# yanyan-li/PlanarSLAM

Hardware: AMD Instinct MI355X
Metric: RGB-D frames/sec (extract+match+pose-opt) @640x480; 1->8-GPU batch scaling (higher is better)
Workload: dtype u8/f64

## Files before the change

planarslam_amd/csrc/planepost.hip:

```cpp
#include "common.h"
#include "isort.h"

#include <algorithm>
#include <cmath>
#include <cstdlib>

namespace planar {
namespace planepost {

#ifndef PLANAR_PP_NT
#define PLANAR_PP_NT 512
#endif
constexpr int NT = PLANAR_PP_NT;
constexpr int MAXP = 128;
constexpr int NRNG = 32768;
constexpr int VOX_BIAS = 8192;
constexpr unsigned long long EMPTY = ~0ull;

struct Geo {
    int dev_skip_heap = 0;
    int pl_first = 0, pl_count = 1 << 20;
    int W, H, max_points, pl_stride, tcap, mini;
    float fx, fy, cx, cy, factor, leaf;
    double dist_th, log_probability, rfx, rfy;
    size_t ws_stride, off_cnt, off_cent, off_key, off_rank, off_vstart, off_pl, off_init, off_meta, off_ranges, off_blocks, off_heapj, off_items, off_dsort, off_gpos;
    int rows_long = 0, gpos_half = 0;
};

struct Pt { float x, y, z; };
__device__ __forceinline__ double mul_rcp(double n, double rd, bool& near) {
    const double t = n * rd;
    const int low = (int)((unsigned)__double_as_longlong(t) & 0x1fffffffu) - 0x10000000;
    near = low >= -8 && low <= 8;
    return t;
}
__device__ __forceinline__ Pt cam_point(const Geo& G, unsigned short d, int px, int py) {
    const double z = (double)d * (double)G.factor;
    const double nx = ((double)px - (double)G.cx) * z, ny = ((double)py - (double)G.cy) * z;
    bool near_x, near_y;
    double tx = mul_rcp(nx, G.rfx, near_x), ty = mul_rcp(ny, G.rfy, near_y);
    if (__ballot(near_x || near_y) != 0ull) {
        if (near_x) tx = nx / (double)G.fx;
        if (near_y) ty = ny / (double)G.fy;
    }
    return {(float)tx, (float)ty, (float)z};
}

__device__ __forceinline__ bool voxel_key(float x, float y, float z, float inv, unsigned plane, unsigned long long& key) {
    const int i0 = (int)floorf(x * inv) + VOX_BIAS, i1 = (int)floorf(y * inv) + VOX_BIAS, i2 = (int)floorf(z * inv) + VOX_BIAS;
    key = ((unsigned long long)plane << 42) | ((unsigned long long)(unsigned)i2 << 28) | ((unsigned long long)(unsigned)i1 << 14) | (unsigned long long)(unsigned)i0;
    return ((unsigned)i0 | (unsigned)i1 | (unsigned)i2) < 2u * VOX_BIAS;
}

__device__ __forceinline__ float red4(float a0, float a1, float a2, float a3) { return (a0 + a2) + (a1 + a3); }
__device__ __forceinline__ float plane_dot(const float m[4], float x, float y, float z) { return red4(m[0] * x, m[1] * y, m[2] * z, m[3] * 1.0f); }

__device__ __forceinline__ void roots2(float b, float c, float roots[3]) {
    roots[0] = 0.f;
    float d = (float)((double)(b * b) - 4.0 * (double)c);
    if (d < 0.0f) d = 0.0f;
    const float sd = sqrtf(d);
    roots[2] = 0.5f * (b + sd);
    roots[1] = 0.5f * (b - sd);
}
__device__ __forceinline__ void roots3(const float m[9], float roots[3]) {
    const float c0 = m[0] * m[4] * m[8] + 2.f * m[1] * m[2] * m[5] - m[0] * m[5] * m[5] - m[4] * m[2] * m[2] - m[8] * m[1] * m[1];
    const float c1 = m[0] * m[4] - m[1] * m[1] + m[0] * m[8] - m[2] * m[2] + m[4] * m[8] - m[5] * m[5];
    const float c2 = m[0] + m[4] + m[8];
    if (fabsf(c0) < 1.1920929e-07f) { roots2(c2, c1, roots); return; }
    const float s_inv3 = (float)(1.0 / 3.0), s_sqrt3 = sqrtf(3.0f);
    const float c2_over_3 = c2 * s_inv3;
    float a_over_3 = (c1 - c2 * c2_over_3) * s_inv3;
    if (a_over_3 > 0.f) a_over_3 = 0.f;
    const float half_b = 0.5f * (c0 + c2_over_3 * (2.f * c2_over_3 * c2_over_3 - c1));
    float q = half_b * half_b + a_over_3 * a_over_3 * a_over_3;
    if (q > 0.f) q = 0.f;
    const float rho = sqrtf(-a_over_3);
    const float theta = atan2f(sqrtf(-q), half_b) * s_inv3;
    const float cos_theta = cosf(theta), sin_theta = sinf(theta);
    roots[0] = c2_over_3 + 2.f * rho * cos_theta;
    roots[1] = c2_over_3 - rho * (cos_theta + s_sqrt3 * sin_theta);
    roots[2] = c2_over_3 - rho * (cos_theta - s_sqrt3 * sin_theta);
    float t;
    if (roots[0] >= roots[1]) { t = roots[0]; roots[0] = roots[1]; roots[1] = t; }
    if (roots[1] >= roots[2]) {
        t = roots[1]; roots[1] = roots[2]; roots[2] = t;
        if (roots[0] >= roots[1]) { t = roots[0]; roots[0] = roots[1]; roots[1] = t; }
    }
    if (roots[0] <= 0) roots2(c2, c1, roots);
}
__device__ __forceinline__ void eigen33_smallest(const float cov[9], float vec[3]) {
    float scale = 0.f;
#pragma unroll
    for (int k = 0; k < 9; k++) scale = fmaxf(scale, fabsf(cov[k]));
    if (scale <= 1.17549435e-38f) scale = 1.0f;
    float m[9];
#pragma unroll
    for (int k = 0; k < 9; k++) m[k] = cov[k] / scale;
    float roots[3];
    roots3(m, roots);
    m[0] -= roots[0]; m[4] -= roots[0]; m[8] -= roots[0];
    float v1[3], v2[3], v3[3];
    v1[0] = m[1] * m[5] - m[2] * m[4]; v1[1] = m[2] * m[3] - m[0] * m[5]; v1[2] = m[0] * m[4] - m[1] * m[3];
    v2[0] = m[1] * m[8] - m[2] * m[7]; v2[1] = m[2] * m[6] - m[0] * m[8]; v2[2] = m[0] * m[7] - m[1] * m[6];
    v3[0] = m[4] * m[8] - m[5] * m[7]; v3[1] = m[5] * m[6] - m[3] * m[8]; v3[2] = m[3] * m[7] - m[4] * m[6];
    const float l1 = v1[0] * v1[0] + (v1[1] * v1[1] + v1[2] * v1[2]), l2 = v2[0] * v2[0] + (v2[1] * v2[1] + v2[2] * v2[2]),
                l3 = v3[0] * v3[0] + (v3[1] * v3[1] + v3[2] * v3[2]);
    if (l1 >= l2 && l1 >= l3) { const float s = sqrtf(l1); vec[0] = v1[0] / s; vec[1] = v1[1] / s; vec[2] = v1[2] / s; }
    else if (l2 >= l1 && l2 >= l3) { const float s = sqrtf(l2); vec[0] = v2[0] / s; vec[1] = v2[1] / s; vec[2] = v2[2] / s; }
    else { const float s = sqrtf(l3); vec[0] = v3[0] / s; vec[1] = v3[1] / s; vec[2] = v3[2] / s; }
}

__device__ __forceinline__ int sac_plane(const Geo& G, const float* __restrict__ pts, int n, unsigned short* shuf, const int* __restrict__ rng, float coef[4], int* info) {
    const int lane = threadIdx.x & 63;
    auto wfence = [&]() { __builtin_amdgcn_fence(__ATOMIC_SEQ_CST, "wavefront"); __builtin_amdgcn_wave_barrier(); };
    for (int i = lane; i < n; i += 64) shuf[i] = (unsigned short)i;
    wfence();
    const double threshold = G.dist_th, one_over_indices = 1.0 / (double)n;
    int iterations = 0, best = -2147483647, draws = 0, bs0 = -1, bs1 = -1, bs2 = -1;
    double k = 1.0;
    unsigned skipped = 0;
    float bm[4] = {0.f, 0.f, 0.f, 0.f};
    bool have = false, exhausted = false;
    auto count_within = [&](const float m[4]) {
        int c = 0;
        for (int i0 = 0; i0 < n; i0 += 64) {
// ... 91 lines not shown
        cov[0] = a[0] - a[6] * a[6]; cov[1] = a[1] - a[6] * a[7]; cov[2] = a[2] - a[6] * a[8];
        cov[4] = a[3] - a[7] * a[7]; cov[5] = a[4] - a[7] * a[8]; cov[8] = a[5] - a[8] * a[8];
        cov[3] = cov[1]; cov[6] = cov[2]; cov[7] = cov[5];
        float v[3];
        eigen33_smallest(cov, v);
        refined[0] = v[0]; refined[1] = v[1]; refined[2] = v[2]; refined[3] = 0.f;
        refined[3] = -1 * red4(refined[0] * a[6], refined[1] * a[7], refined[2] * a[8], refined[3] * 1.0f);
    }
    const int nref = count_within(refined);
    if (info && lane == 0) { info[5] = n_inl; info[6] = nref; }
#pragma unroll
    for (int c = 0; c < 4; c++) coef[c] = refined[c];
    return nref != 0 ? 0 : 2;
}

__device__ __forceinline__ int max_point_distance(const Geo& G, float plane[4], const float* __restrict__ pts, int n, unsigned short* shuf, const int* __restrict__ rng, int* info) {
    const int lane = threadIdx.x & 63;
    bool far = false;
    for (int i0 = 0; i0 < n; i0 += 64) {
        const int i = i0 + lane;
        bool f = false;
        if (i < n) f = (double)fabsf(plane[0] * pts[i * 3] + plane[1] * pts[i * 3 + 1] + plane[2] * pts[i * 3 + 2] + plane[3]) > G.dist_th;
        far = far || (__ballot(f) != 0ull);
    }
    if (info && lane == 0) for (int c = 0; c < 12; c++) info[c] = c >= 2 && c <= 4 ? -1 : 0;
    if (far) return 1;
    float c[4];
    const int st = sac_plane(G, pts, n, shuf, rng, c, info);
    if (st) return st;
    const float oldVal = plane[3], newVal = c[3];
    const bool flip = (newVal < 0 && oldVal > 0) || (newVal > 0 && oldVal < 0);
#pragma unroll
    for (int t = 0; t < 4; t++) plane[t] = flip ? -c[t] : c[t];
    return 0;
}

__device__ __forceinline__ unsigned hash64(unsigned long long k) {
    k ^= k >> 33; k *= 0xff51afd7ed558ccdull; k ^= k >> 33;
    return (unsigned)k;
}

__device__ __forceinline__ void bitonic(unsigned long long* a, int n2) {
    for (int k = 2; k <= n2; k <<= 1)
        for (int j = k >> 1; j > 0; j >>= 1) {
            for (int t = threadIdx.x; t < n2 / 2; t += NT) {
                const int lo = ((t / j) * 2 * j) + (t % j), hi = lo + j;
                const bool up = (lo & k) == 0;
                const unsigned long long x = a[lo], y = a[hi];
                if ((x > y) == up) { a[lo] = y; a[hi] = x; }
            }
            __syncthreads();
        }
}

#ifndef PLANAR_WIDE_T
#define PLANAR_WIDE_T 1024
#endif
constexpr int PS_T = PLANAR_WIDE_T, PS_LT = 256, PS_E = 23, PS_SHIFT = 19, PS_R = 96;
constexpr int PS_HJOBS = 1024;
struct HeapClass { int max_len, cap, waves, wgs; };
constexpr HeapClass PS_HC[3] = {{2048, 2048, 4, 1}, {8192, 8192, 1, 2}, {1 << 30, 8192, 1, 4}};
using PsLds = isort::LdsLayout<PS_LT, PS_E>;
using PsGl = isort::GlobalLayout<PS_T>;
constexpr int PS_IT_SMALL = 256, PS_IT_BATCH = 256;
constexpr int ERR_SORT = 5;

struct Meta { int n_init, counts[2], err, M, npl, sort_status, heap_n, heap_n_global; };

__global__ __launch_bounds__(NT) void plane_voxels_kernel(Geo G, const unsigned short* __restrict__ depth_all, int pitch_px, long frame_stride_px,
                                                          const int* __restrict__ labels_all, const int* __restrict__ n_planes, unsigned char* ws_all, long long* timing) {
    extern __shared__ unsigned long long s_list[];
    __shared__ int s_first[MAXP], s_last[MAXP];
    __shared__ int s_n, s_err, s_kept, s_scan[NT / 64];
    const int b = blockIdx.x, tid = threadIdx.x, lane = tid & 63, wave = tid >> 6;
    const int HW = G.W * G.H;
    const unsigned short* D = depth_all + (size_t)b * frame_stride_px;
    const int* lab = labels_all + (size_t)b * HW;
    unsigned char* ws = ws_all + (size_t)b * G.ws_stride;
    unsigned* tcnt = (unsigned*)(ws + G.off_cnt);
    unsigned long long* gkey = (unsigned long long*)(ws + G.off_key);
    unsigned short* srank = (unsigned short*)(ws + G.off_rank);
    int* vstart = (int*)(ws + G.off_vstart);
    int* pfl = (int*)(ws + G.off_pl);
    isort::Range* init = (isort::Range*)(ws + G.off_init);
    Meta* meta = (Meta*)(ws + G.off_meta);
    int npl = n_planes[b];
    if (npl > MAXP) npl = MAXP;
    if (npl > G.pl_stride) npl = G.pl_stride;
    const float inv = 1.0f / G.leaf;
    const int TC = G.tcap;
    long long* tmark = timing ? timing + (size_t)b * 16 : nullptr;
    auto mark = [&](int q) { if (tmark && tid == 0) tmark[q] = wall_clock64(); };
    mark(0);

    for (int i = tid; i < TC; i += NT) { gkey[i] = EMPTY; tcnt[i] = 0u; }
    for (int i = tid; i < MAXP; i += NT) { s_first[i] = 0; s_last[i] = 0; }
    if (tid == 0) { s_n = 0; s_err = 0; s_kept = 0; }
    __threadfence();
    __syncthreads();

    mark(1);
    {
        constexpr int ROWS = 60, UNR = 4;
        const int MINI = G.mini;
        unsigned long long* mk = s_list + (size_t)wave * MINI;
        unsigned* mc = (unsigned*)(s_list + (size_t)(NT / 64) * MINI) + (size_t)wave * MINI;
        auto wfence = [&]() { __builtin_amdgcn_fence(__ATOMIC_SEQ_CST, "wavefront"); __builtin_amdgcn_wave_barrier(); };
        auto to_frame = [&](unsigned long long key, unsigned cnt) {
            unsigned h = hash64(key) & (unsigned)(TC - 1);
            for (int probe = 0; probe < TC; probe++) {
                const unsigned long long k = atomicCAS(&gkey[h], EMPTY, key);
                if (k == EMPTY) { if (atomicAdd(&s_n, 1) >= G.max_points) s_err = 3; }
                if (k == EMPTY || k == key) { atomicAdd(&tcnt[h], cnt); return; }
                h = (h + 1) & (unsigned)(TC - 1);
            }
            s_err = 3;
        };
        const int strips = (G.W + 63) / 64, tiles = strips * ((G.H + ROWS - 1) / ROWS);
        for (int tile = wave; tile < tiles; tile += NT / 64) {
            const int px = (tile % strips) * 64 + lane, y0 = (tile / strips) * ROWS, y1 = min(y0 + ROWS, G.H);
            const bool col = px < G.W;
            for (int e = lane; e < MINI; e += 64) { mk[e] = EMPTY; mc[e] = 0u; }
            wfence();
            unsigned long long cur = EMPTY, pend = EMPTY;
            unsigned cnt = 0, pcnt = 0;
            auto flush_parked = [&]() {
                if (pend != EMPTY) {
                    unsigned h = (hash64(pend) >> 7) & (unsigned)(MINI - 1);
                    bool done = false;
                    for (int probe = 0; probe < 8 && !done; probe++) {
                        const unsigned long long k = atomicCAS(&mk[h], EMPTY, pend);
                        if (k == EMPTY || k == pend) { atomicAdd(&mc[h], pcnt); done = true; }
                        h = (h + 1) & (unsigned)(MINI - 1);
                    }
                    if (!done) to_frame(pend, pcnt);
                    pend = EMPTY;
                }
            };
            int l4[UNR], ln[UNR];
            unsigned short d4[UNR], dn[UNR];
            const int pxc = min(px, G.W - 1);
            auto load = [&](int yb, int* l, unsigned short* d) {
#pragma unroll
                for (int q = 0; q < UNR; q++) {
                    const int yy = min(yb + q, G.H - 1);
                    const int lv = lab[(size_t)yy * G.W + pxc];
                    d[q] = D[(size_t)yy * pitch_px + pxc];
                    l[q] = (col && yb + q < y1) ? lv : -1;
                }
            };
            load(y0, l4, d4);
            for (int yb = y0; yb < y1; yb += UNR) {
                load(yb + UNR, ln, dn);
#pragma unroll
                for (int q = 0; q < UNR; q++) {
                    const int l = l4[q];
                    const bool on = l >= G.pl_first && l < npl && l - G.pl_first < G.pl_count;
                    unsigned long long key = cur;
                    bool fin = false;
                    const Pt p = cam_point(G, d4[q], px, yb + q);
                    if (on) {
                        if (!voxel_key(p.x, p.y, p.z, inv, (unsigned)l, key)) { s_err = 3; key = cur; }
                        fin = key != cur;
                    }
                    if (__ballot(fin && cur != EMPTY && pend != EMPTY) != 0ull) flush_parked();
                    if (fin) {
                        if (cur != EMPTY) { pend = cur; pcnt = cnt; }
                        cur = key; cnt = 0;
                    }
                    if (on && key == cur && cur != EMPTY) cnt++;
                }
#pragma unroll
                for (int q = 0; q < UNR; q++) { l4[q] = ln[q]; d4[q] = dn[q]; }
            }
            flush_parked();
            pend = cur; pcnt = cnt;
            flush_parked();
            wfence();
            for (int e = lane; e < MINI; e += 64)
                if (mk[e] != EMPTY) to_frame(mk[e], mc[e]);
            wfence();
        }
    }
    __threadfence();
    __syncthreads();
    const int err = s_err;
    const int M = err ? 0 : s_n;
    mark(2);

    if (!err) {
        int n2 = 64;
        while (n2 < M) n2 <<= 1;
        if (tid == 0) s_kept = 0;
        for (int i = M + tid; i < n2; i += NT) s_list[i] = EMPTY;
        __syncthreads();
        for (int i = tid; i < TC; i += NT) {
            const unsigned long long k = __hip_atomic_load(&gkey[i], __ATOMIC_RELAXED, __HIP_MEMORY_SCOPE_AGENT);
            if (k != EMPTY) s_list[atomicAdd(&s_kept, 1)] = (k << 14) | (unsigned long long)i;
        }
        __syncthreads();
        bitonic(s_list, n2);
        const int per = (M + NT - 1) / NT, r0 = min(M, tid * per), r1 = min(M, r0 + per);
        int mine = 0;
        for (int r = r0; r < r1; r++) {
            const unsigned long long e = s_list[r];
            const int s = (int)(e & 0x3fffull), p = (int)(e >> 56);
            srank[s] = (unsigned short)r;
            mine += (int)__hip_atomic_load(&tcnt[s], __ATOMIC_RELAXED, __HIP_MEMORY_SCOPE_AGENT);
            if (r == 0 || (int)(s_list[r - 1] >> 56) != p) s_first[p] = r;
            if (r == M - 1 || (int)(s_list[r + 1] >> 56) != p) s_last[p] = r + 1;
        }
        int total;
        int run = isort::block_exscan<NT, int>(mine, s_scan, &total);
        for (int r = r0; r < r1; r++) {
            vstart[r] = run;
            run += (int)__hip_atomic_load(&tcnt[(int)(s_list[r] & 0x3fffull)], __ATOMIC_RELAXED, __HIP_MEMORY_SCOPE_AGENT);
        }
        if (tid == 0) vstart[M] = total;
    }
    __threadfence();
    __syncthreads();
    for (int p = tid; p < MAXP; p += NT) { pfl[p] = s_first[p]; pfl[MAXP + p] = s_last[p]; }
    if (tid == 0) {
        int k = 0;
        for (int p = 0; p < npl && !err; p++) {
            if (s_last[p] <= s_first[p]) continue;
            const int f = vstart[s_first[p]], l = vstart[s_last[p]];
            init[k++] = isort::Range{f, l, isort::depth_limit(l - f)};
        }
        meta->n_init = k; meta->counts[0] = 0; meta->counts[1] = 0; meta->err = err; meta->M = M; meta->npl = npl; meta->sort_status = 0; meta->heap_n = 0; meta->heap_n_global = 0;
    }
    mark(3);
}

template <int SH, int IT>
__global__ __launch_bounds__(IT) void plane_items_kernel(Geo G, const unsigned short* __restrict__ depth_all, int pitch_px, long frame_stride_px,
                                                           const int* __restrict__ labels_all, unsigned char* ws_all) {
    constexpr int NW = IT / 64;
    __shared__ unsigned s_cnt[NW][MAXP];
    const int b = blockIdx.x, tid = threadIdx.x, lane = tid & 63, wave = tid >> 6;
    const int HW = G.W * G.H;
    unsigned char* ws = ws_all + (size_t)b * G.ws_stride;
    const Meta* meta = (const Meta*)(ws + G.off_meta);
    if (meta->err || meta->n_init == 0) return;
    const unsigned short* D = depth_all + (size_t)b * frame_stride_px;
    const int* lab = labels_all + (size_t)b * HW;
    const unsigned long long* gkey = (const unsigned long long*)(ws + G.off_key);
    const unsigned short* srank = (const unsigned short*)(ws + G.off_rank);
    const int* vstart = (const int*)(ws + G.off_vstart);
    const int* pfl = (const int*)(ws + G.off_pl);
    uint32_t* items = (uint32_t*)(ws + G.off_items);
    const int npl = meta->npl, TC = G.tcap;
    const float inv = 1.0f / G.leaf;
    for (int i = tid; i < NW * MAXP; i += IT) (&s_cnt[0][0])[i] = 0u;
    __syncthreads();
    const int S = ((HW + NW - 1) / NW + 63) & ~63, w0 = min(HW, wave * S), w1 = min(HW, w0 + S);
    auto wfence = [&]() { __builtin_amdgcn_fence(__ATOMIC_SEQ_CST, "wavefront"); __builtin_amdgcn_wave_barrier(); };
    constexpr int U = 4;
    for (int i0 = w0; i0 < w1; i0 += 64 * U) {
        int l[U];
#pragma unroll
        for (int u = 0; u < U; u++) l[u] = lab[min(i0 + 64 * u + lane, w1 - 1)];
#pragma unroll
        for (int u = 0; u < U; u++) {
            const bool on = i0 + 64 * u + lane < w1 && l[u] >= G.pl_first && l[u] < npl && l[u] - G.pl_first < G.pl_count;
            unsigned long long rem = __ballot(on);
            while (rem) {
                const int L = __builtin_amdgcn_readlane(l[u], __builtin_ctzll(rem));
                const unsigned long long m = __ballot(on && l[u] == L);
                if (lane == 0) s_cnt[wave][L] += (unsigned)__popcll(m);
                rem &= ~m;
            }
        }
    }
    __syncthreads();
    if (tid < npl) {
        const int first = pfl[tid], last = pfl[MAXP + tid];
        unsigned run = last > first ? (unsigned)vstart[first] : 0u;
        for (int w = 0; w < NW; w++) { const unsigned t = s_cnt[w][tid]; s_cnt[w][tid] = run; run += t; }
    }
    __syncthreads();
    for (int i0 = w0; i0 < w1; i0 += 64 * U) {
        int l[U];
        unsigned short d[U];
#pragma unroll
        for (int u = 0; u < U; u++) {
            const int pix = min(i0 + 64 * u + lane, w1 - 1), py = pix / G.W, px = pix - py * G.W;
            l[u] = lab[pix];
            d[u] = D[(size_t)py * pitch_px + px];
        }
#pragma unroll
        for (int u = 0; u < U; u++) {
            const int pix = i0 + 64 * u + lane, pc = min(pix, w1 - 1), py = pc / G.W, px = pc - py * G.W;
            const bool on = pix < w1 && l[u] >= G.pl_first && l[u] < npl && l[u] - G.pl_first < G.pl_count;
            const Pt p = cam_point(G, d[u], px, py);
            uint32_t item = 0;
            if (on) {
                unsigned long long key;
                voxel_key(p.x, p.y, p.z, inv, (unsigned)l[u], key);
                unsigned h = hash64(key) & (unsigned)(TC - 1);
                for (int probe = 0; probe < TC && gkey[h] != key; probe++) h = (h + 1) & (unsigned)(TC - 1);
                item = ((uint32_t)srank[h] << SH) | (uint32_t)pix;
            }
            unsigned long long rem = __ballot(on);
            while (rem) {
                const int L = __builtin_amdgcn_readlane(l[u], __builtin_ctzll(rem));
                const bool mine = on && l[u] == L;
                const unsigned long long m = __ballot(mine);
                const unsigned base = s_cnt[wave][L];
                wfence();
                if (mine) items[base + (unsigned)__popcll(m & ((1ull << lane) - 1ull))] = item;
                if (lane == 0) s_cnt[wave][L] = base + (unsigned)__popcll(m);
                wfence();
                rem &= ~m;
            }
        }
    }
}

template <int SH>
__global__ __launch_bounds__(PS_T) void plane_sort_global(Geo G, unsigned char* ws_all, int rows_cap) {
    extern __shared__ __align__(16) uint8_t sort_lds[];
    unsigned char* ws = ws_all + (size_t)blockIdx.x * G.ws_stride;
    Meta* meta = (Meta*)(ws + G.off_meta);
    if (meta->err || meta->n_init == 0) return;
    const isort::HeapSink HS{(isort::HeapJob*)(ws + G.off_heapj), &meta->heap_n, PS_HJOBS};
    isort::global_tier<SH, PS_T>((uint32_t*)(ws + G.off_items), (const isort::Range*)(ws + G.off_init), meta->n_init, PsLds::N, 64, (isort::Range*)(ws + G.off_ranges),
                                 (isort::Block*)(ws + G.off_blocks), isort::G_FMAX, meta->counts, sort_lds, rows_cap, HS, &meta->sort_status, 0xffffffffu,
                                 G.rows_long, G.rows_long ? (uint32_t*)(ws + G.off_gpos) : nullptr, G.gpos_half);
    __syncthreads();
    if (threadIdx.x == 0) meta->heap_n_global = min(meta->heap_n, PS_HJOBS);
}

constexpr int PS_EARLY = 4;
template <int SH>
__global__ __launch_bounds__(PS_LT, 4) void plane_sort_lds(Geo G, unsigned char* ws_all) {
    extern __shared__ __align__(16) uint8_t sort_lds[];
    unsigned char* ws = ws_all + (size_t)blockIdx.x * G.ws_stride;
    Meta* meta = (Meta*)(ws + G.off_meta);
    if (meta->err) return;
    if (blockIdx.y < PS_EARLY) {
        static_assert(PsLds::bytes >= PS_HC[2].cap * 4, "the early heap jobs keep the top PS_HC[2].cap words of a range in this workgroup's LDS");
        const int ng = meta->heap_n_global;
        if (threadIdx.x < 64 && ng > 0 && !G.dev_skip_heap)
            isort::heap_jobs<SH>((uint32_t*)(ws + G.off_items), (const isort::HeapJob*)(ws + G.off_heapj), ng, blockIdx.y, PS_EARLY, (uint32_t*)sort_lds, PS_HC[2].cap, 0, 1 << 30);
        return;
    }
    const isort::Range* ranges = (const isort::Range*)(ws + G.off_ranges);
    const isort::Block* blocks = (const isort::Block*)(ws + G.off_blocks);
    const int nb = meta->counts[1];
    const isort::HeapSink HS{(isort::HeapJob*)(ws + G.off_heapj), &meta->heap_n, PS_HJOBS};
    for (int k = blockIdx.y - PS_EARLY; k < nb; k += gridDim.y - PS_EARLY) {
        const isort::Block K = blocks[k];
        isort::lds_tier<SH, PS_LT, PS_E>((uint32_t*)(ws + G.off_items), ranges + K.r0, K.nr, K.f, K.l, sort_lds, HS, &meta->sort_status);
    }
}

template <int SH>
__global__ __launch_bounds__(256) void plane_sort_heap(Geo G, unsigned char* ws_all, int part, int min_len, int max_len, int cap) {
    extern __shared__ __align__(16) uint8_t sort_lds[];
    unsigned char* ws = ws_all + (size_t)blockIdx.x * G.ws_stride;
    const Meta* meta = (const Meta*)(ws + G.off_meta);
    const int ng = meta->heap_n_global, lo = part ? ng : 0, hi = meta->err ? 0 : (part ? min(meta->heap_n, PS_HJOBS) : ng), wave = threadIdx.x >> 6, nw = blockDim.x >> 6;
    if (hi > lo) isort::heap_jobs<SH>((uint32_t*)(ws + G.off_items), (const isort::HeapJob*)(ws + G.off_heapj) + lo, hi - lo, blockIdx.y * nw + wave, gridDim.y * nw,
                                           (uint32_t*)sort_lds + (size_t)wave * cap, cap, min_len, max_len);
}

__device__ __forceinline__ Pt cam_point_thread(const Geo& G, unsigned short d, int px, int py) {
    const double z = (double)d * (double)G.factor;
    const double nx = ((double)px - (double)G.cx) * z, ny = ((double)py - (double)G.cy) * z;
    bool near_x, near_y;
    double tx = mul_rcp(nx, G.rfx, near_x), ty = mul_rcp(ny, G.rfy, near_y);
    if (near_x) tx = nx / (double)G.fx;
    if (near_y) ty = ny / (double)G.fy;
    return {(float)tx, (float)ty, (float)z};
}

template <int SH>
__global__ __launch_bounds__(NT, 4) void plane_tail_kernel(Geo G, const unsigned short* __restrict__ depth_all, int pitch_px, long frame_stride_px,
                                                        const double* __restrict__ planes_all, int planes_stride, const int* __restrict__ rng, unsigned char* ws_all,
                                                        int* n_out, float* coef_out, int* src_out, int* off_out, float* pts_out, int* status, int* state_out,
                                                        int* nvox_out, int* info_out, long long* timing) {
    extern __shared__ unsigned long long s_list[];
    __shared__ int s_first[MAXP], s_last[MAXP], s_state[MAXP], s_k[MAXP], s_o[MAXP + 1];
    __shared__ float s_coef[MAXP][4];
    __shared__ int s_err, s_kept;
    const int b = blockIdx.x, tid = threadIdx.x, lane = tid & 63, wave = tid >> 6;
    const unsigned short* D = depth_all + (size_t)b * frame_stride_px;
    const double* planes = planes_all + (size_t)b * planes_stride * 8;
    unsigned char* ws = ws_all + (size_t)b * G.ws_stride;
    float* cent = (float*)(ws + G.off_cent);
    const int* vstart = (const int*)(ws + G.off_vstart);
    const int* pfl = (const int*)(ws + G.off_pl);
    const uint32_t* items = (const uint32_t*)(ws + G.off_items);
    const Meta* meta = (const Meta*)(ws + G.off_meta);
    const int npl = meta->npl;
    int err = meta->err ? meta->err : (meta->sort_status ? ERR_SORT : 0);
    const int M = err ? 0 : meta->M;
    long long* tmark = timing ? timing + (size_t)b * 16 : nullptr;
    auto mark = [&](int q) { if (tmark && tid == 0) tmark[q] = wall_clock64(); };
    for (int i = tid; i < MAXP; i += NT) { s_first[i] = pfl[i]; s_last[i] = pfl[MAXP + i]; s_state[i] = (i >= G.pl_first && i - G.pl_first < G.pl_count) ? 0 : 3; }
    if (tid == 0) { s_err = 0; s_kept = 0; }
    {
        unsigned short* dsort = (unsigned short*)(ws + G.off_dsort);
        const int total = M > 0 ? vstart[M] : 0;
        for (int i = tid; i < total; i += NT) {
            const int pix = (int)(items[i] & ((1u << SH) - 1u)), yy = pix / G.W;
            dsort[i] = D[(size_t)yy * pitch_px + (pix - yy * G.W)];
        }
        __threadfence_block();
        __syncthreads();
        for (int r = tid; r < M; r += NT) {
            const int i0 = vstart[r], i1 = vstart[r + 1];
            float cx = 0.f, cy = 0.f, cz = 0.f;
            constexpr int U = 16;
            for (int i = i0; i < i1; i += U) {
                uint32_t it[U];
                unsigned short d[U];
#pragma unroll
                for (int u = 0; u < U; u++) { it[u] = items[min(i + u, i1 - 1)]; d[u] = dsort[min(i + u, i1 - 1)]; }
#pragma unroll
                for (int u = 0; u < U; u++)
                    if (i + u < i1) {
                        const int pix = (int)(it[u] & ((1u << SH) - 1u)), yy = pix / G.W;
                        const Pt p = cam_point_thread(G, d[u], pix - yy * G.W, yy);
                        cx += p.x; cy += p.y; cz += p.z;
                    }
            }
            const float cnt = (float)(i1 - i0);
            cent[(size_t)r * 3] = cx / cnt; cent[(size_t)r * 3 + 1] = cy / cnt; cent[(size_t)r * 3 + 2] = cz / cnt;
        }
    }
    __threadfence();
    __syncthreads();

    mark(3);
    unsigned short* shuf = (unsigned short*)s_list;
    if (!err)
    for (int p = wave; p < npl; p += NT / 64) {
        if (s_state[p] != 0) continue;
        const double* P = planes + (size_t)p * 8;
        const double nx = P[1], ny = P[2], nz = P[3];
        float c[4] = {(float)nx, (float)ny, (float)nz, (float)-(nx * P[4] + ny * P[5] + nz * P[6])};
        const int first = s_first[p], n = s_last[p] - first;
        int* info = info_out ? info_out + ((size_t)b * G.pl_stride + p) * 12 : nullptr;
        const int st = max_point_distance(G, c, cent + (size_t)first * 3, n, shuf + first, rng, info);
        if (lane == 0) {
            s_state[p] = st;
#pragma unroll
            for (int t = 0; t < 4; t++) s_coef[p][t] = c[t];
            if (st == 4) s_err = 4;
        }
    }
    __syncthreads();
    if (!err) err = s_err;
    mark(4);

// ... 150 lines not shown
    const int* vstart = (const int*)(ws + G.off_vstart);
    const uint32_t* items = (const uint32_t*)(ws + G.off_items);
    const Meta* meta = (const Meta*)(ws + G.off_meta);
    const int err = meta->err ? meta->err : (meta->sort_status ? ERR_SORT : 0), M = err ? 0 : meta->M;
    for (int r = tid; r < M; r += NT) {
        const int i0 = vstart[r], i1 = vstart[r + 1];
        float cx = 0.f, cy = 0.f, cz = 0.f;
        for (int i = i0; i < i1; i++) { const int j = (int)(items[i] & ((1u << PS_SHIFT) - 1u)); cx += pts[j * 3]; cy += pts[j * 3 + 1]; cz += pts[j * 3 + 2]; }
        const float cnt = (float)(i1 - i0);
        out[(size_t)r * 3] = cx / cnt; out[(size_t)r * 3 + 1] = cy / cnt; out[(size_t)r * 3 + 2] = cz / cnt;
    }
    if (tid == 0) { *n_out = M; *status = err; }
}

static void sampler_table(std::vector<int>& tab) {
    std::vector<uint32_t> s(624);
    s[0] = 12345u;
    for (int i = 1; i < 624; i++) s[i] = 1812433253u * (s[i - 1] ^ (s[i - 1] >> 30)) + (uint32_t)i;
    int at = 624;
    tab.resize(NRNG);
    for (int q = 0; q < NRNG; q++) {
        if (at >= 624) {
            for (int i = 0; i < 624; i++) {
                const uint32_t y = (s[i] & 0x80000000u) | (s[(i + 1) % 624] & 0x7fffffffu);
                s[i] = s[(i + 397) % 624] ^ (y >> 1) ^ ((y & 1u) ? 0x9908b0dfu : 0u);
            }
            at = 0;
        }
        uint32_t y = s[at++];
        y ^= y >> 11; y ^= (y << 7) & 0x9d2c5680u; y ^= (y << 15) & 0xefc60000u; y ^= y >> 18;
        tab[q] = (int)(y >> 1);
    }
}

}
}

struct planar_plane_clouds {
    planar_ctx* ctx = nullptr;
    int max_batch = 0;
    planar::planepost::Geo G{};
    size_t smem = 0, smem_tail = 0, smem_cloud = 0, smem_sort_g = 0, smem_sort_l = 0;
    int sort_rows = 0, shift = 19;
    planar::DevBuf ws, rng, dbg;
    bool timing = false;
    std::vector<int32_t> last_status;
    planar::LaunchProfile prof{6};
};

using namespace planar;

extern "C" {

int planar_plane_clouds_create(planar_ctx* ctx, int width, int height, int max_batch, int max_points, planar_plane_clouds** out) {
    PLANAR_REQUIRE(ctx && out, PLANAR_EINVAL, "null argument");
    PLANAR_REQUIRE(width >= 16 && height >= 16 && width <= 4096 && height <= 4096 && max_batch >= 1, PLANAR_EINVAL, "bad size");
    PLANAR_REQUIRE(max_points >= 64 && max_points <= 8192 && (max_points & (max_points - 1)) == 0, PLANAR_EINVAL, "max_points must be a power of two in [64, 8192]");
    PLANAR_REQUIRE((long long)width * height <= (1ll << 20), PLANAR_EINVAL, "at most 2^20 pixels per frame (a sort word is voxel << 20 | pixel)");
    PLANAR_REQUIRE((long long)width * height <= (1ll << planepost::PS_SHIFT) || max_points <= 4096, PLANAR_EINVAL, "frames of more than 2^19 pixels take max_points <= 4096 (12 bits of voxel beside 20 bits of pixel)");
    PLANAR_HIP_CHECK(hipSetDevice(ctx->device));
    planar_plane_clouds* p = new planar_plane_clouds;
    p->ctx = ctx; p->max_batch = max_batch;
    planepost::Geo& G = p->G;
    G.W = width; G.H = height; G.max_points = max_points; G.pl_stride = planepost::MAXP;
    G.leaf = 0.1f; G.dist_th = 0.05;
    G.log_probability = std::log(1.0 - 0.99);
    G.tcap = 2 * max_points;
    {
        size_t off = 0;
        auto carve = [&](size_t bytes) { const size_t o = off; off = align_up(off + bytes, (size_t)256); return o; };
        G.off_cnt = carve((size_t)G.tcap * 4);
        G.off_key = carve((size_t)G.tcap * 8);
        G.off_rank = carve((size_t)G.tcap * 2);
        G.off_cent = carve((size_t)max_points * 12);
        G.off_vstart = carve((size_t)(max_points + 1) * 4);
        G.off_pl = carve((size_t)2 * planepost::MAXP * 4);
        G.off_init = carve((size_t)planepost::MAXP * sizeof(isort::Range));
        G.off_meta = carve(sizeof(planepost::Meta));
        G.off_ranges = carve((size_t)isort::G_FMAX * sizeof(isort::Range));
        G.off_blocks = carve((size_t)isort::G_FMAX * sizeof(isort::Block));
        G.off_heapj = carve((size_t)planepost::PS_HJOBS * sizeof(isort::HeapJob));
        G.off_items = carve(std::max((size_t)width * height, (size_t)65536) * 4);
        G.off_dsort = carve((size_t)width * height * 2);
        if (!planepost::PsGl::plan(std::max(width * height, 65536), p->sort_rows, G.rows_long)) { delete p; set_error("plane_clouds: frame too large for the sort's LDS-resident rank prefixes"); return PLANAR_EINVAL; }
        G.gpos_half = G.rows_long ? width * height / 2 + 2 : 0;
        G.off_gpos = carve(G.rows_long ? (size_t)G.gpos_half * 2 * 4 : 0);
        G.ws_stride = off;
    }
    p->shift = (long long)width * height <= (1ll << planepost::PS_SHIFT) ? planepost::PS_SHIFT : 20;
    G.mini = 128;
    p->smem = std::max((size_t)(planepost::NT / 64) * G.mini * 12, (size_t)max_points * 8);
    p->smem_tail = (size_t)max_points * 2;
    p->smem_cloud = (size_t)G.tcap * 8;
    p->smem_sort_g = (size_t)planepost::PsGl::bytes(p->sort_rows);
    p->smem_sort_l = (size_t)planepost::PsLds::bytes;
    int rc = p->ws.alloc(G.ws_stride * (size_t)max_batch);
    if (!rc) rc = p->rng.alloc((size_t)planepost::NRNG * 4);
    if (rc) { delete p; return rc; }
    std::vector<int> tab;
    planepost::sampler_table(tab);
    if (hipMemcpy(p->rng.p, tab.data(), tab.size() * 4, hipMemcpyHostToDevice) != hipSuccess) { set_error("plane_clouds: sampler table upload failed"); delete p; return PLANAR_EDEVICE; }
    {
        hipError_t e = hipSuccess;
        if (p->smem > 40 * 1024) e = hipFuncSetAttribute((const void*)planepost::plane_voxels_kernel, hipFuncAttributeMaxDynamicSharedMemorySize, (int)p->smem);
        if (e == hipSuccess && p->smem_cloud > 40 * 1024) e = hipFuncSetAttribute((const void*)planepost::cloud_voxels_kernel, hipFuncAttributeMaxDynamicSharedMemorySize, (int)p->smem_cloud);
        if (e == hipSuccess) e = hipFuncSetAttribute((const void*)planepost::plane_sort_global<19>, hipFuncAttributeMaxDynamicSharedMemorySize, (int)p->smem_sort_g);
        if (e == hipSuccess) e = hipFuncSetAttribute((const void*)planepost::plane_sort_lds<19>, hipFuncAttributeMaxDynamicSharedMemorySize, (int)p->smem_sort_l);
        if (e == hipSuccess) e = hipFuncSetAttribute((const void*)planepost::plane_sort_heap<19>, hipFuncAttributeMaxDynamicSharedMemorySize, planepost::PS_HC[2].cap * 4);
        if (e == hipSuccess) e = hipFuncSetAttribute((const void*)planepost::plane_sort_global<20>, hipFuncAttributeMaxDynamicSharedMemorySize, (int)p->smem_sort_g);
        if (e == hipSuccess) e = hipFuncSetAttribute((const void*)planepost::plane_sort_lds<20>, hipFuncAttributeMaxDynamicSharedMemorySize, (int)p->smem_sort_l);
        if (e == hipSuccess) e = hipFuncSetAttribute((const void*)planepost::plane_sort_heap<20>, hipFuncAttributeMaxDynamicSharedMemorySize, planepost::PS_HC[2].cap * 4);
        if (e != hipSuccess) { (void)hipGetLastError(); set_error("plane_clouds: %zu bytes of LDS per workgroup are not available", std::max(std::max(p->smem, p->smem_cloud), p->smem_sort_g)); delete p; return PLANAR_EINVAL; }
    }
    *out = p;
    return PLANAR_OK;
}

void planar_plane_clouds_destroy(planar_plane_clouds* p) { delete p; }

int planar_plane_clouds_set_plane_window(planar_plane_clouds* p, int first, int count) {
    PLANAR_REQUIRE(p && first >= 0, PLANAR_EINVAL, "bad argument");
    p->G.pl_first = count < 0 ? 0 : first;
    p->G.pl_count = count < 0 ? (1 << 20) : count;
    return PLANAR_OK;
}

int planar_plane_clouds_set_timing(planar_plane_clouds* p, int enable) {
    PLANAR_REQUIRE(p != nullptr, PLANAR_EINVAL, "null argument");
    if (enable && !p->dbg.p) { int rc = p->dbg.alloc((size_t)p->max_batch * 128); if (rc) return rc; }
    p->timing = enable != 0;
    return PLANAR_OK;
}
int planar_plane_clouds_read_timing(planar_plane_clouds* p, int B, int64_t* out) {
    PLANAR_REQUIRE(p && out && p->dbg.p && B >= 1 && B <= p->max_batch, PLANAR_EINVAL, "timing not enabled / bad B");
    PLANAR_HIP_CHECK(hipStreamSynchronize(p->ctx->stream));
    PLANAR_HIP_CHECK(hipMemcpy(out, p->dbg.p, (size_t)B * 128, hipMemcpyDeviceToHost));
    return PLANAR_OK;
}

int planar_plane_clouds_set_profiling(planar_plane_clouds* p, int enable) {
    PLANAR_REQUIRE(p != nullptr, PLANAR_EINVAL, "null argument");
    PLANAR_HIP_CHECK(hipStreamSynchronize(p->ctx->stream));
    p->prof.on = enable != 0;
    p->prof.reset();
    return PLANAR_OK;
}
int planar_plane_clouds_get_profile(planar_plane_clouds* p, double* total_ms , int64_t* calls) {
    PLANAR_REQUIRE(p && total_ms && calls, PLANAR_EINVAL, "null argument");
    PLANAR_HIP_CHECK(hipStreamSynchronize(p->ctx->stream));
    return p->prof.sum(total_ms, calls);
}

int planar_plane_clouds_sort_stats(planar_plane_clouds* p, int B, int64_t* out ) {
    PLANAR_REQUIRE(p && out && B >= 1 && B <= p->max_batch, PLANAR_EINVAL, "bad argument");
    PLANAR_HIP_CHECK(hipSetDevice(p->ctx->device));
    PLANAR_HIP_CHECK(hipStreamSynchronize(p->ctx->stream));
    std::vector<isort::HeapJob> jobs(planepost::PS_HJOBS);
    for (int b = 0; b < B; b++) {
        const unsigned char* ws = p->ws.as<unsigned char>() + (size_t)b * p->G.ws_stride;
        planepost::Meta m;
        PLANAR_HIP_CHECK(hipMemcpy(&m, ws + p->G.off_meta, sizeof(m), hipMemcpyDeviceToHost));
        const int nj = std::min(m.heap_n, planepost::PS_HJOBS);
        if (nj) PLANAR_HIP_CHECK(hipMemcpy(jobs.data(), ws + p->G.off_heapj, (size_t)nj * sizeof(isort::HeapJob), hipMemcpyDeviceToHost));
        int64_t el = 0, mx = 0;
        for (int j = 0; j < nj; j++) { el += jobs[j].l - jobs[j].f; mx = std::max<int64_t>(mx, jobs[j].l - jobs[j].f); }
        out[b * 4] = m.heap_n; out[b * 4 + 1] = el; out[b * 4 + 2] = mx; out[b * 4 + 3] = m.counts[1];
    }
    return PLANAR_OK;
}

int planar_plane_clouds_stride(const planar_plane_clouds* p, int* pl_stride, int* max_points) {
    PLANAR_REQUIRE(p != nullptr, PLANAR_EINVAL, "null argument");
    if (pl_stride) *pl_stride = p->G.pl_stride;
    if (max_points) *max_points = p->G.max_points;
    return PLANAR_OK;
}

int planar_plane_clouds_compute_dev(planar_plane_clouds* p, const uint16_t* d_depth, int B, int pitch_px, int64_t frame_stride_px, float fx, float fy, float cx,
                                    float cy, float depth_factor, const int32_t* d_labels, const double* d_planes, const int32_t* d_n_planes, double dist_th,
                                    float leaf, int32_t* d_n_out, float* d_coef, int32_t* d_src, int32_t* d_pt_off, float* d_points, int32_t* d_status,
                                    int32_t* d_state, int32_t* d_nvox, int32_t* d_info) {
    PLANAR_REQUIRE(p && d_depth && d_labels && d_planes && d_n_planes && d_n_out && d_coef && d_src && d_pt_off && d_points && d_status, PLANAR_EINVAL, "null argument");
    PLANAR_REQUIRE(B >= 1 && B <= p->max_batch, PLANAR_EINVAL, "B must be in [1, max_batch]");
    PLANAR_REQUIRE(pitch_px >= p->G.W && frame_stride_px >= (int64_t)pitch_px * p->G.H, PLANAR_EINVAL, "pitch/frame_stride too small");
    PLANAR_REQUIRE(leaf > 0.f && dist_th >= 0.0, PLANAR_EINVAL, "leaf / dist_th");
    planepost::Geo G = p->G;
    G.fx = fx; G.fy = fy; G.cx = cx; G.cy = cy; G.factor = depth_factor; G.leaf = leaf; G.dist_th = dist_th;
    G.rfx = 1.0 / (double)fx; G.rfy = 1.0 / (double)fy;
    hipStream_t st = p->ctx->stream;
    unsigned char* ws = p->ws.as<unsigned char>();
    long long* tm = p->timing ? p->dbg.as<long long>() : nullptr;
    const int rc = p->prof.begin();
    if (rc) return rc;
    auto mark = [&]() { p->prof.mark(st); };
    mark();
    hipLaunchKernelGGL(planepost::plane_voxels_kernel, dim3(B), dim3(planepost::NT), p->smem, st, G, d_depth, pitch_px, (long)frame_stride_px, d_labels, d_n_planes, ws, tm);
    mark();
#define PLANAR_BY_SHIFT(K, ...) do { if (p->shift == 20) hipLaunchKernelGGL(planepost::K<20>, __VA_ARGS__); else hipLaunchKernelGGL(planepost::K<19>, __VA_ARGS__); } while (0)
    if (B >= planepost::PS_IT_BATCH) {
        if (p->shift == 20) hipLaunchKernelGGL((planepost::plane_items_kernel<20, planepost::PS_IT_SMALL>), dim3(B), dim3(planepost::PS_IT_SMALL), 0, st, G, d_depth, pitch_px, (long)frame_stride_px, d_labels, ws);
        else hipLaunchKernelGGL((planepost::plane_items_kernel<19, planepost::PS_IT_SMALL>), dim3(B), dim3(planepost::PS_IT_SMALL), 0, st, G, d_depth, pitch_px, (long)frame_stride_px, d_labels, ws);
    } else {
        if (p->shift == 20) hipLaunchKernelGGL((planepost::plane_items_kernel<20, planepost::PS_T>), dim3(B), dim3(planepost::PS_T), 0, st, G, d_depth, pitch_px, (long)frame_stride_px, d_labels, ws);
        else hipLaunchKernelGGL((planepost::plane_items_kernel<19, planepost::PS_T>), dim3(B), dim3(planepost::PS_T), 0, st, G, d_depth, pitch_px, (long)frame_stride_px, d_labels, ws);
    }
    mark();
    PLANAR_BY_SHIFT(plane_sort_global, dim3(B), dim3(planepost::PS_T), p->smem_sort_g, st, G, ws, p->sort_rows);
    mark();
    auto heap_launch = [&](hipStream_t q, int part, int c) {
        const planepost::HeapClass& H = planepost::PS_HC[c];
        PLANAR_BY_SHIFT(plane_sort_heap, dim3(B, H.wgs), dim3(64 * H.waves), (size_t)H.cap * 4 * H.waves, q, G, ws, part, c ? planepost::PS_HC[c - 1].max_len + 1 : 0, H.max_len, H.cap);
    };
    PLANAR_BY_SHIFT(plane_sort_lds, dim3(B, planepost::PS_EARLY + planepost::PS_R), dim3(planepost::PS_LT), p->smem_sort_l, st, G, ws);
    mark();
    heap_launch(st, 1, 0); heap_launch(st, 1, 1);
    mark();
    PLANAR_BY_SHIFT(plane_tail_kernel, dim3(B), dim3(planepost::NT), p->smem_tail, st, G, d_depth, pitch_px, (long)frame_stride_px, d_planes,
                    planar_peac_max_planes(), p->rng.as<int>(), ws, d_n_out, d_coef, d_src, d_pt_off, d_points, d_status, d_state, d_nvox, d_info, tm);
#undef PLANAR_BY_SHIFT
    mark();
    PLANAR_HIP_CHECK(hipGetLastError());
    return PLANAR_OK;
}

int planar_plane_clouds_compute(planar_plane_clouds* p, const uint16_t* depth, int B, int pitch_px, int64_t frame_stride_px, float fx, float fy, float cx, float cy,
                                float depth_factor, const int32_t* labels, const double* planes, const int32_t* n_planes, double dist_th, float leaf, int32_t* n_out,
                                float* coef, int32_t* src, int32_t* pt_off, float* points, int32_t* state, int32_t* nvox, int32_t* info) {
    PLANAR_REQUIRE(p && depth && labels && planes && n_planes && n_out && coef && src && pt_off && points, PLANAR_EINVAL, "null argument");
    PLANAR_REQUIRE(B >= 1 && B <= p->max_batch, PLANAR_EINVAL, "B must be in [1, max_batch]");
    PLANAR_REQUIRE(pitch_px >= p->G.W && frame_stride_px >= (int64_t)pitch_px * p->G.H, PLANAR_EINVAL, "pitch/frame_stride too small");
    PLANAR_HIP_CHECK(hipSetDevice(p->ctx->device));
    const int PS = p->G.pl_stride, MP = p->G.max_points, HW = p->G.W * p->G.H;
    Stager s;
    const size_t nb = (size_t)B;
    const auto d_depth = s.in(depth, (size_t)frame_stride_px * (B - 1) + (size_t)pitch_px * p->G.H);
    const auto d_lab = s.in(labels, nb * HW);
    const auto d_pl = s.in(planes, nb * planar_peac_max_planes() * 8);
    const auto d_np = s.in(n_planes, nb);
    const auto o_n = s.out(n_out, nb);
    const auto o_coef = s.out(coef, nb * PS * 4);
    const auto o_src = s.out(src, nb * PS), o_off = s.out(pt_off, nb * (PS + 1));
    const auto o_pts = s.out(points, nb * MP * 3);
    std::vector<int32_t> h_status(B);
    const auto o_st = s.out(h_status.data(), nb), o_state = s.out(state, nb * PS), o_nvox = s.out(nvox, nb * PS), o_info = s.out(info, nb * PS * 12);
    hipStream_t st = p->ctx->stream;
    int rc = s.upload(st);
    if (rc) return rc;
    PLANAR_HIP_CHECK(s.zero_from(o_n, st));
    if ((rc = planar_plane_clouds_compute_dev(p, d_depth, B, pitch_px, frame_stride_px, fx, fy, cx, cy, depth_factor, d_lab, d_pl, d_np, dist_th, leaf, o_n, o_coef, o_src, o_off,
                                              o_pts, o_st, o_state, o_nvox, o_info)))
        return rc;
    if ((rc = s.download(st))) return rc;
    p->last_status = h_status;
    for (int b = 0; b < B; b++)
        if (h_status[b]) { set_error("plane_clouds: frame %d exceeded a capacity (code %d: 3 = voxels / index range, 4 = sampler table, 5 = the std::sort order of a plane's points is not reproducible: introsort depth limit / sort workspace)", b, h_status[b]); return PLANAR_ECAPACITY; }
    return PLANAR_OK;
}

int planar_plane_clouds_last_status(planar_plane_clouds* p, int B, int32_t* out) {
    PLANAR_REQUIRE(p && out && B >= 1, PLANAR_EINVAL, "bad argument");
    PLANAR_REQUIRE((size_t)B <= p->last_status.size(), PLANAR_EINVAL, "the last planar_plane_clouds_compute call had fewer frames");
    for (int b = 0; b < B; b++) out[b] = p->last_status[b];
    return PLANAR_OK;
}

int planar_plane_refit(planar_plane_clouds* p, int n_clouds, const float* points, const int32_t* pt_off, double dist_th, float* planes, int32_t* state, int32_t* info) {
    PLANAR_REQUIRE(p && points && pt_off && planes && state, PLANAR_EINVAL, "null argument");
    PLANAR_REQUIRE(n_clouds >= 1, PLANAR_EINVAL, "n_clouds");
    PLANAR_HIP_CHECK(hipSetDevice(p->ctx->device));
    int max_n = 0;
    for (int q = 0; q < n_clouds; q++) { PLANAR_REQUIRE(pt_off[q + 1] >= pt_off[q], PLANAR_EINVAL, "pt_off must be non-decreasing"); max_n = std::max(max_n, pt_off[q + 1] - pt_off[q]); }
    PLANAR_REQUIRE(max_n <= 32768 && pt_off[0] == 0, PLANAR_EINVAL, "a cloud may hold at most 32768 points");
    Stager s;
    const auto d_pts = s.in(points, (size_t)pt_off[n_clouds] * 3);
    const auto d_off = s.in(pt_off, (size_t)n_clouds + 1);
    const auto io_pl = s.inout(planes, (size_t)n_clouds * 4);
    const auto o_st = s.out(state, (size_t)n_clouds), o_info = s.out(info, (size_t)n_clouds * 12);
    hipStream_t st = p->ctx->stream;
    int rc = s.upload(st);
    if (rc) return rc;
    planepost::Geo G = p->G;
    G.dist_th = dist_th;
    const size_t smem = align_up((size_t)std::max(max_n, 1) * 2, (size_t)16);
    if (smem > 40 * 1024) PLANAR_HIP_CHECK(hipFuncSetAttribute((const void*)planepost::refit_kernel, hipFuncAttributeMaxDynamicSharedMemorySize, (int)smem));
    hipLaunchKernelGGL(planepost::refit_kernel, dim3(n_clouds), dim3(64), smem, st, G, n_clouds, d_pts, d_off, p->rng.as<int>(), io_pl, o_st, o_info);
    PLANAR_HIP_CHECK(hipGetLastError());
    return s.download(st);
// ... 68 lines not shown
```

Before: 12650.

## Precompute per-band plane counts in voxel kernel to make item pass single-sweep

The voxel kernel now accumulates per-wave, per-plane point counts in LDS and flushes them into a per-row-band global table. The items kernel reads these band counts to seed its per-wave offsets, so its separate counting sweep over all pixels is removed. Its per-wave pixel ranges are realigned to band boundaries, and the block is sized to the number of bands. The hash lookups are batched across unrolled pixels and only run for run-head lanes, with the rank broadcast to the other lanes. It also stores camera intrinsics as doubles. The cost is extra LDS atomics and global band-table atomics in the voxel kernel, and more LDS.

Result: no change. 12610 (-0.3%).

```diff
diff --git a/planarslam_amd/csrc/planepost.hip b/planarslam_amd/csrc/planepost.hip
--- a/planarslam_amd/csrc/planepost.hip
+++ b/planarslam_amd/csrc/planepost.hip
@@ -15,6 +15,7 @@
 constexpr int MAXP = 128;
 constexpr int NRNG = 32768;
 constexpr int VOX_BIAS = 8192;
+constexpr int BAND_ROWS = 60;
 constexpr unsigned long long EMPTY = ~0ull;
 
 struct Geo {
@@ -23,7 +24,9 @@
     int W, H, max_points, pl_stride, tcap, mini;
     float fx, fy, cx, cy, factor, leaf;
     double dist_th, log_probability, rfx, rfy;
-    size_t ws_stride, off_cnt, off_cent, off_key, off_rank, off_vstart, off_pl, off_init, off_meta, off_ranges, off_blocks, off_heapj, off_items, off_dsort, off_gpos;
+    double dfx, dfy, dcx, dcy, dfactor;
+    size_t ws_stride, off_cnt, off_cent, off_key, off_rank, off_vstart, off_pl, off_init, off_meta, off_ranges, off_blocks, off_heapj, off_items, off_dsort, off_gpos, off_band;
+    int bands = 0;
     int rows_long = 0, gpos_half = 0;
 };
 
@@ -35,13 +38,13 @@
     return t;
 }
 __device__ __forceinline__ Pt cam_point(const Geo& G, unsigned short d, int px, int py) {
-    const double z = (double)d * (double)G.factor;
-    const double nx = ((double)px - (double)G.cx) * z, ny = ((double)py - (double)G.cy) * z;
+    const double z = (double)d * G.dfactor;
+    const double nx = ((double)px - G.dcx) * z, ny = ((double)py - G.dcy) * z;
     bool near_x, near_y;
     double tx = mul_rcp(nx, G.rfx, near_x), ty = mul_rcp(ny, G.rfy, near_y);
     if (__ballot(near_x || near_y) != 0ull) {
-        if (near_x) tx = nx / (double)G.fx;
-        if (near_y) ty = ny / (double)G.fy;
+        if (near_x) tx = nx / G.dfx;
+        if (near_y) ty = ny / G.dfy;
     }
     return {(float)tx, (float)ty, (float)z};
 }
@@ -299,6 +302,7 @@
     unsigned short* srank = (unsigned short*)(ws + G.off_rank);
     int* vstart = (int*)(ws + G.off_vstart);
     int* pfl = (int*)(ws + G.off_pl);
+    unsigned* bandcnt = (unsigned*)(ws + G.off_band);
     isort::Range* init = (isort::Range*)(ws + G.off_init);
     Meta* meta = (Meta*)(ws + G.off_meta);
     int npl = n_planes[b];
@@ -311,19 +315,26 @@
     mark(0);
 
     for (int i = tid; i < TC; i += NT) { gkey[i] = EMPTY; tcnt[i] = 0u; }
+    for (int i = tid; i < G.bands * MAXP; i += NT) bandcnt[i] = 0u;
     for (int i = tid; i < MAXP; i += NT) { s_first[i] = 0; s_last[i] = 0; }
+    {
+        unsigned* pc_all = (unsigned*)(s_list + (size_t)(NT / 64) * G.mini) + (size_t)(NT / 64) * G.mini;
+        for (int i = tid; i < (NT / 64) * MAXP; i += NT) pc_all[i] = 0u;
+    }
     if (tid == 0) { s_n = 0; s_err = 0; s_kept = 0; }
     __threadfence();
     __syncthreads();
 
     mark(1);
     {
-        constexpr int ROWS = 60, UNR = 4;
+        constexpr int ROWS = BAND_ROWS, UNR = 4;
         const int MINI = G.mini;
         unsigned long long* mk = s_list + (size_t)wave * MINI;
         unsigned* mc = (unsigned*)(s_list + (size_t)(NT / 64) * MINI) + (size_t)wave * MINI;
+        unsigned* pc = (unsigned*)(s_list + (size_t)(NT / 64) * MINI) + (size_t)(NT / 64) * MINI + (size_t)wave * MAXP;
         auto wfence = [&]() { __builtin_amdgcn_fence(__ATOMIC_SEQ_CST, "wavefront"); __builtin_amdgcn_wave_barrier(); };
         auto to_frame = [&](unsigned long long key, unsigned cnt) {
+            atomicAdd(&pc[(unsigned)(key >> 42)], cnt);
             unsigned h = hash64(key) & (unsigned)(TC - 1);
             for (int probe = 0; probe < TC; probe++) {
                 const unsigned long long k = atomicCAS(&gkey[h], EMPTY, key);
@@ -397,6 +408,11 @@
             for (int e = lane; e < MINI; e += 64)
                 if (mk[e] != EMPTY) to_frame(mk[e], mc[e]);
             wfence();
+            for (int e = lane; e < npl; e += 64) {
+                const unsigned c = pc[e];
+                if (c) { atomicAdd(&bandcnt[(size_t)(tile / strips) * MAXP + e], c); pc[e] = 0u; }
+            }
+            wfence();
         }
     }
     __threadfence();
@@ -451,11 +467,10 @@
 }
 
 template <int SH, int IT>
-__global__ __launch_bounds__(IT) void plane_items_kernel(Geo G, const unsigned short* __restrict__ depth_all, int pitch_px, long frame_stride_px,
+__global__ __launch_bounds__(IT, IT <= 256 ? 8 : 4) void plane_items_kernel(Geo G, const unsigned short* __restrict__ depth_all, int pitch_px, long frame_stride_px,
                                                            const int* __restrict__ labels_all, unsigned char* ws_all) {
-    constexpr int NW = IT / 64;
-    __shared__ unsigned s_cnt[NW][MAXP];
-    const int b = blockIdx.x, tid = threadIdx.x, lane = tid & 63, wave = tid >> 6;
+    __shared__ unsigned s_cnt[IT / 64][MAXP];
+    const int b = blockIdx.x, tid = threadIdx.x, lane = tid & 63, wave = tid >> 6, NW = (int)blockDim.x >> 6;
     const int HW = G.W * G.H;
     unsigned char* ws = ws_all + (size_t)b * G.ws_stride;
     const Meta* meta = (const Meta*)(ws + G.off_meta);
@@ -466,63 +481,81 @@
     const unsigned short* srank = (const unsigned short*)(ws + G.off_rank);
     const int* vstart = (const int*)(ws + G.off_vstart);
     const int* pfl = (const int*)(ws + G.off_pl);
+    const unsigned* bandcnt = (const unsigned*)(ws + G.off_band);
     uint32_t* items = (uint32_t*)(ws + G.off_items);
     const int npl = meta->npl, TC = G.tcap;
     const float inv = 1.0f / G.leaf;
-    for (int i = tid; i < NW * MAXP; i += IT) (&s_cnt[0][0])[i] = 0u;
+    if (tid < npl) {
+        const int first = pfl[tid], last = pfl[MAXP + tid];
+        unsigned run = last > first ? (unsigned)vstart[first] : 0u;
+        for (int w = 0; w < NW; w++) {
+            s_cnt[w][tid] = run;
+            for (int k = w * G.bands / NW; k < (w + 1) * G.bands / NW; k++) run += bandcnt[(size_t)k * MAXP + tid];
+        }
+    }
     __syncthreads();
-    const int S = ((HW + NW - 1) / NW + 63) & ~63, w0 = min(HW, wave * S), w1 = min(HW, w0 + S);
+    const int w0 = min(HW, (wave * G.bands / NW) * BAND_ROWS * G.W), w1 = min(HW, ((wave + 1) * G.bands / NW) * BAND_ROWS * G.W);
     auto wfence = [&]() { __builtin_amdgcn_fence(__ATOMIC_SEQ_CST, "wavefront"); __builtin_amdgcn_wave_barrier(); };
     constexpr int U = 4;
     for (int i0 = w0; i0 < w1; i0 += 64 * U) {
         int l[U];
-#pragma unroll
-        for (int u = 0; u < U; u++) l[u] = lab[min(i0 + 64 * u + lane, w1 - 1)];
+        {
+            int lv[U];
+            unsigned short d[U];
+#pragma unroll
+            for (int u = 0; u < U; u++) {
+                const int pix = min(i0 + 64 * u + lane, w1 - 1), py = pix / G.W, px = pix - py * G.W;
+                lv[u] = lab[pix];
+                d[u] = D[(size_t)py * pitch_px + px];
+            }
+#pragma unroll
+            for (int u = 0; u < U; u++) {
+                const bool on = i0 + 64 * u + lane < w1 && lv[u] >= G.pl_first && lv[u] < npl && lv[u] - G.pl_first < G.pl_count;
+                l[u] = on ? ((int)d[u] << 8) | lv[u] : -1;
+            }
+        }
+        unsigned h[U];
+        unsigned long long key[U];
+        bool head[U], need[U];
 #pragma unroll
         for (int u = 0; u < U; u++) {
-            const bool on = i0 + 64 * u + lane < w1 && l[u] >= G.pl_first && l[u] < npl && l[u] - G.pl_first < G.pl_count;
+            const int pc = min(i0 + 64 * u + lane, w1 - 1), py = pc / G.W, px = pc - py * G.W;
+            const bool on = l[u] >= 0;
+            const Pt p = cam_point(G, (unsigned short)(l[u] >> 8), px, py);
+            l[u] = on ? l[u] & 0xff : -1;
+            key[u] = EMPTY;
+            if (on) voxel_key(p.x, p.y, p.z, inv, (unsigned)l[u], key[u]);
+            const unsigned plo = (unsigned)__builtin_amdgcn_update_dpp(-1, (int)(unsigned)key[u], 0x138, 0xf, 0xf, false);
+            const unsigned phi = (unsigned)__builtin_amdgcn_update_dpp(-1, (int)(unsigned)(key[u] >> 32), 0x138, 0xf, 0xf, false);
+            head[u] = on && (lane == 0 || (((unsigned long long)phi << 32) | plo) != key[u]);
+            need[u] = head[u];
+            h[u] = hash64(key[u]) & (unsigned)(TC - 1);
+        }
+        for (int probe = 0; probe < TC; probe++) {
+            unsigned long long k[U];
+#pragma unroll
+            for (int u = 0; u < U; u++) if (need[u]) k[u] = gkey[h[u]];
+            bool more = false;
+#pragma unroll
+            for (int u = 0; u < U; u++)
+                if (need[u]) {
+                    if (k[u] == key[u]) need[u] = false;
+                    else { h[u] = (h[u] + 1) & (unsigned)(TC - 1); more = true; }
+                }
+            if (__ballot(more) == 0ull) break;
+        }
+#pragma unroll
+        for (int u = 0; u < U; u++) {
+            const int pix = i0 + 64 * u + lane;
+            const bool on = l[u] >= 0;
+            int r = head[u] ? (int)srank[h[u]] : 0;
+            const unsigned long long heads = __ballot(head[u]) | 1ull;
+            r = __shfl(r, 63 - __builtin_clzll(heads & (~0ull >> (63 - lane))));
+            const uint32_t item = ((uint32_t)r << SH) | (uint32_t)pix;
             unsigned long long rem = __ballot(on);
             while (rem) {
                 const int L = __builtin_amdgcn_readlane(l[u], __builtin_ctzll(rem));
-                const unsigned long long m = __ballot(on && l[u] == L);
-                if (lane == 0) s_cnt[wave][L] += (unsigned)__popcll(m);
-                rem &= ~m;
-            }
-        }
-    }
-    __syncthreads();
-    if (tid < npl) {
-        const int first = pfl[tid], last = pfl[MAXP + tid];
-        unsigned run = last > first ? (unsigned)vstart[first] : 0u;
-        for (int w = 0; w < NW; w++) { const unsigned t = s_cnt[w][tid]; s_cnt[w][tid] = run; run += t; }
-    }
-    __syncthreads();
-    for (int i0 = w0; i0 < w1; i0 += 64 * U) {
-        int l[U];
-        unsigned short d[U];
-#pragma unroll
-        for (int u = 0; u < U; u++) {
-            const int pix = min(i0 + 64 * u + lane, w1 - 1), py = pix / G.W, px = pix - py * G.W;
-            l[u] = lab[pix];
-            d[u] = D[(size_t)py * pitch_px + px];
-        }
-#pragma unroll
-        for (int u = 0; u < U; u++) {
-            const int pix = i0 + 64 * u + lane, pc = min(pix, w1 - 1), py = pc / G.W, px = pc - py * G.W;
-            const bool on = pix < w1 && l[u] >= G.pl_first && l[u] < npl && l[u] - G.pl_first < G.pl_count;
-            const Pt p = cam_point(G, d[u], px, py);
-            uint32_t item = 0;
-            if (on) {
-                unsigned long long key;
-                voxel_key(p.x, p.y, p.z, inv, (unsigned)l[u], key);
-                unsigned h = hash64(key) & (unsigned)(TC - 1);
-                for (int probe = 0; probe < TC && gkey[h] != key; probe++) h = (h + 1) & (unsigned)(TC - 1);
-                item = ((uint32_t)srank[h] << SH) | (uint32_t)pix;
-            }
-            unsigned long long rem = __ballot(on);
-            while (rem) {
-                const int L = __builtin_amdgcn_readlane(l[u], __builtin_ctzll(rem));
-                const bool mine = on && l[u] == L;
+                const bool mine = l[u] == L;
                 const unsigned long long m = __ballot(mine);
                 const unsigned base = s_cnt[wave][L];
                 wfence();
@@ -584,12 +617,12 @@
 }
 
 __device__ __forceinline__ Pt cam_point_thread(const Geo& G, unsigned short d, int px, int py) {
-    const double z = (double)d * (double)G.factor;
-    const double nx = ((double)px - (double)G.cx) * z, ny = ((double)py - (double)G.cy) * z;
+    const double z = (double)d * G.dfactor;
+    const double nx = ((double)px - G.dcx) * z, ny = ((double)py - G.dcy) * z;
     bool near_x, near_y;
     double tx = mul_rcp(nx, G.rfx, near_x), ty = mul_rcp(ny, G.rfy, near_y);
-    if (near_x) tx = nx / (double)G.fx;
-    if (near_y) ty = ny / (double)G.fy;
+    if (near_x) tx = nx / G.dfx;
+    if (near_y) ty = ny / G.dfy;
     return {(float)tx, (float)ty, (float)z};
 }
 
@@ -906,6 +939,8 @@
         G.off_heapj = carve((size_t)planepost::PS_HJOBS * sizeof(isort::HeapJob));
         G.off_items = carve(std::max((size_t)width * height, (size_t)65536) * 4);
         G.off_dsort = carve((size_t)width * height * 2);
+        G.bands = (height + planepost::BAND_ROWS - 1) / planepost::BAND_ROWS;
+        G.off_band = carve((size_t)G.bands * planepost::MAXP * 4);
         if (!planepost::PsGl::plan(std::max(width * height, 65536), p->sort_rows, G.rows_long)) { delete p; set_error("plane_clouds: frame too large for the sort's LDS-resident rank prefixes"); return PLANAR_EINVAL; }
         G.gpos_half = G.rows_long ? width * height / 2 + 2 : 0;
         G.off_gpos = carve(G.rows_long ? (size_t)G.gpos_half * 2 * 4 : 0);
@@ -913,7 +948,7 @@
     }
     p->shift = (long long)width * height <= (1ll << planepost::PS_SHIFT) ? planepost::PS_SHIFT : 20;
     G.mini = 128;
-    p->smem = std::max((size_t)(planepost::NT / 64) * G.mini * 12, (size_t)max_points * 8);
+    p->smem = std::max((size_t)(planepost::NT / 64) * (G.mini * 12 + planepost::MAXP * 4), (size_t)max_points * 8);
     p->smem_tail = (size_t)max_points * 2;
     p->smem_cloud = (size_t)G.tcap * 8;
     p->smem_sort_g = (size_t)planepost::PsGl::bytes(p->sort_rows);
@@ -1011,6 +1046,7 @@
     planepost::Geo G = p->G;
     G.fx = fx; G.fy = fy; G.cx = cx; G.cy = cy; G.factor = depth_factor; G.leaf = leaf; G.dist_th = dist_th;
     G.rfx = 1.0 / (double)fx; G.rfy = 1.0 / (double)fy;
+    G.dfx = (double)fx; G.dfy = (double)fy; G.dcx = (double)cx; G.dcy = (double)cy; G.dfactor = (double)depth_factor;
     hipStream_t st = p->ctx->stream;
     unsigned char* ws = p->ws.as<unsigned char>();
     long long* tm = p->timing ? p->dbg.as<long long>() : nullptr;
@@ -1025,8 +1061,9 @@
         if (p->shift == 20) hipLaunchKernelGGL((planepost::plane_items_kernel<20, planepost::PS_IT_SMALL>), dim3(B), dim3(planepost::PS_IT_SMALL), 0, st, G, d_depth, pitch_px, (long)frame_stride_px, d_labels, ws);
         else hipLaunchKernelGGL((planepost::plane_items_kernel<19, planepost::PS_IT_SMALL>), dim3(B), dim3(planepost::PS_IT_SMALL), 0, st, G, d_depth, pitch_px, (long)frame_stride_px, d_labels, ws);
     } else {
-        if (p->shift == 20) hipLaunchKernelGGL((planepost::plane_items_kernel<20, planepost::PS_T>), dim3(B), dim3(planepost::PS_T), 0, st, G, d_depth, pitch_px, (long)frame_stride_px, d_labels, ws);
-        else hipLaunchKernelGGL((planepost::plane_items_kernel<19, planepost::PS_T>), dim3(B), dim3(planepost::PS_T), 0, st, G, d_depth, pitch_px, (long)frame_stride_px, d_labels, ws);
+        const int it = 64 * std::min(planepost::PS_T / 64, G.bands);
+        if (p->shift == 20) hipLaunchKernelGGL((planepost::plane_items_kernel<20, planepost::PS_T>), dim3(B), dim3(it), 0, st, G, d_depth, pitch_px, (long)frame_stride_px, d_labels, ws);
+        else hipLaunchKernelGGL((planepost::plane_items_kernel<19, planepost::PS_T>), dim3(B), dim3(it), 0, st, G, d_depth, pitch_px, (long)frame_stride_px, d_labels, ws);
     }
     mark();
     PLANAR_BY_SHIFT(plane_sort_global, dim3(B), dim3(planepost::PS_T), p->smem_sort_g, st, G, ws, p->sort_rows);
```
